# jisang93/VISinger

Hardware: AMD Instinct MI355X
Metric: audio samples/sec (22.05 kHz) + flow log-det rel-err, B=32 T_mel=1024 (higher is better)
Workload: dtype f32 (split-f16 x3 on the f16 MFMA, f32 accumulate); 1 GPU; VISinger synthesis (text-enc + pitch-pred + frame-prior + flow-inverse + HiFi-GAN), B=32/GPU T_mel=1024 hop=256 hidden=192 fp32 tensors, random-init weights; per_gpu_batch=32, global_batch=32, t_mel=1024, hop=256, hidden=192, parallelism=dp1 (utterance shard, no collective), streams=2

## Files before the change

visinger_amd/csrc/resblock_f16.hip:

```cpp
#include "conv_common.h"

#include <algorithm>
#include <type_traits>

namespace vs {

__device__ __forceinline__ unsigned max3_u32(unsigned a, unsigned b, unsigned c) {
    unsigned r;
    asm("v_max3_u32 %0, %1, %2, %3" : "=v"(r) : "v"(a), "v"(b), "v"(c));
    return r;
}

typedef float f32x4 __attribute__((ext_vector_type(4)));

#ifdef VS_RB_MFMA32
constexpr bool RB_MFMA16 = false;
#else
constexpr bool RB_MFMA16 = true;
#endif

constexpr int RB_MAXCONV = 6;
constexpr int RB_MAXPAD = 28;

struct ResblockParams {
    const float *x;
    long long x_bs;
    const void *ws[RB_MAXCONV];
    const float *bias[RB_MAXCONV];
    const float *wscale[RB_MAXCONV];
    int dil[RB_MAXCONV];
    float *y;
    const float *acc;
    long long y_bs, acc_bs;
    float scale;
    int B, C, T, K, nconv, nchunks;
    int H;
    int MP;
    int fast_epi;
    int bf16;
    unsigned long long *stamps;
};

__device__ __forceinline__ void rb_stamp(const ResblockParams &p, int slot) {
    if (p.stamps && threadIdx.x == 0) {
        const unsigned lin = blockIdx.x + gridDim.x * blockIdx.z;
        p.stamps[(size_t)lin * 64 + slot] = __builtin_amdgcn_s_memrealtime();
        p.stamps[(size_t)lin * 64 + 32 + slot] = __builtin_amdgcn_s_memtime();
    }
}

template <int NT_W, int WAVES_M, int WAVES_N, int MP, int PLANES, bool PB>
__device__ __forceinline__ void resblock_body(const ResblockParams &p) {
    constexpr int NW = WAVES_M * WAVES_N;
    static_assert(NW == 4 || NW == 8, "four or eight waves");
    static_assert(PLANES == 2 || (PLANES == 1), "two f16 planes or one bf16 plane");
    static_assert(!PB || PLANES == 1, "bf16-resident tensors go with the plain-bf16 arithmetic");
    constexpr int BN = 32 * NT_W * WAVES_N;
    constexpr int KG = 4 * WAVES_M;
    constexpr int WT = BN + 2 * MP;
    constexpr int TPL = KG * WT * 4;
    extern __shared__ __attribute__((aligned(16))) float smem[];
    unsigned *const Tb = reinterpret_cast<unsigned *>(smem);
    int *const smax = reinterpret_cast<int *>(Tb + PLANES * TPL);

    const int tid = threadIdx.x, lane = tid & 63;
    const int wave = __builtin_amdgcn_readfirstlane(tid >> 6);
    const int wm = wave % WAVES_M, wn = wave / WAVES_M;
    constexpr bool M16 = RB_MFMA16 && PLANES == 2;
    constexpr int NA = M16 ? 4 * NT_W : NT_W, AR = M16 ? 4 : 16;
    constexpr int NCT = M16 ? 2 * NT_W : NT_W, CTW = M16 ? 16 : 32;
    constexpr int RT = M16 ? 2 : 1;
    constexpr int KSTEP = M16 ? 32 : 16;
    using acc_t = std::conditional_t<M16, f32x4, f32x16>;
    auto ct_of = [](int a) { return M16 ? (a >> 1) : a; };
    const int lhalf = lane >> 5;
    const int lcol = lane & (CTW - 1);
    auto tile_col = [&](int a) { return ct_of(a) * CTW + lcol; };
    const int b = blockIdx.z;
    const int NOUT = BN - 2 * p.H;
    const int n0 = blockIdx.x * NOUT;
    const int t0 = n0 - p.H;
    const int KT = p.K;
    const int nch = p.nchunks / (KSTEP / 16);
    const int nsteps = nch * KT;
    auto tile_row = [&](int a, int r) { return M16 ? 16 * (a & 1) + 4 * (lane >> 4) + r : (r & 3) + 8 * (r >> 2) + 4 * lhalf; };

    rb_stamp(p, 0);
    for (int e = tid; e < PLANES * KG * 2 * MP; e += 64 * NW) {
        const int rowi = e / (2 * MP), c = e % (2 * MP);
        *reinterpret_cast<u32x4 *>(Tb + (rowi * WT + (c < MP ? c : BN + c)) * 4) = u32x4{0u, 0u, 0u, 0u};
    }

    bool inside[NCT];
    acc_t xr[NA], acc[NA];
    {
        const char *const xbase = reinterpret_cast<const char *>(p.x) + (long long)b * p.x_bs * (PB ? 2 : 4);
        const __amdgpu_buffer_rsrc_t xsrc =
            __builtin_amdgcn_make_buffer_rsrc((void *)xbase, 0, (int)((long long)p.C * p.T * (PB ? 2 : 4)), 0x00020000);
#pragma unroll
        for (int j = 0; j < NCT; ++j) {
            const int n = t0 + wn * (NT_W * 32) + j * CTW + lcol;
            inside[j] = (n >= 0) && (n < p.T);
        }
#pragma unroll
        for (int a = 0; a < NA; ++a) {
            const int nc = min(max(t0 + wn * (NT_W * 32) + tile_col(a), 0), p.T - 1);
#pragma unroll
            for (int r = 0; r < AR; ++r) {
                if constexpr (PB)
                    xr[a][r] = u2f((unsigned)(unsigned short)__builtin_amdgcn_raw_buffer_load_b16(xsrc, ((wm * 32 + tile_row(a, r)) * p.T + nc) * 2, 0, 0) << 16);
                else
                    xr[a][r] = __builtin_bit_cast(float, __builtin_amdgcn_raw_buffer_load_b32(xsrc, ((wm * 32 + tile_row(a, r)) * p.T + nc) * 4, 0, 0));
            }
        }
#pragma unroll
        for (int a = 0; a < NA; ++a)
#pragma unroll
            for (int r = 0; r < AR; ++r) xr[a][r] = inside[ct_of(a)] ? xr[a][r] : 0.f;
    }

    bool all_in = true;
#pragma unroll
    for (int j = 0; j < NCT; ++j) all_in = all_in && (__builtin_amdgcn_ballot_w64(inside[j]) == ~0ull);
    rb_stamp(p, 1);
    auto mma_step = [&](const u32x4 (&acur)[RT][PLANES], const unsigned *xs, auto zc_c) __attribute__((always_inline)) {
        constexpr bool ZC = decltype(zc_c)::value;
        const f32x16 zero16 = {0.f, 0.f, 0.f, 0.f, 0.f, 0.f, 0.f, 0.f, 0.f, 0.f, 0.f, 0.f, 0.f, 0.f, 0.f, 0.f};
        const f32x4 zero4 = {0.f, 0.f, 0.f, 0.f};
        u32x4 bf[PLANES], bn[PLANES];
#pragma unroll
        for (int pl = 0; pl < PLANES; ++pl) bf[pl] = *reinterpret_cast<const u32x4 *>(xs + pl * TPL);
#pragma unroll
        for (int j = 0; j < NCT; ++j) {
            if (j + 1 < NCT) {
#pragma unroll
                for (int pl = 0; pl < PLANES; ++pl) bn[pl] = *reinterpret_cast<const u32x4 *>(xs + pl * TPL + (j + 1) * (CTW * 4));
            }
            __builtin_amdgcn_sched_barrier(0);
            if constexpr (M16) {
                auto mm = [&](int ta, int tb) __attribute__((always_inline)) {
#pragma unroll
                    for (int rt = 0; rt < 2; ++rt)
                        acc[2 * j + rt] = __builtin_amdgcn_mfma_f32_16x16x32_f16(__builtin_bit_cast(f16x8, acur[rt][ta]), __builtin_bit_cast(f16x8, bf[tb]), acc[2 * j + rt], 0, 0, 0);
                };
                if constexpr (ZC) {
#pragma unroll
                    for (int rt = 0; rt < 2; ++rt)
                        acc[2 * j + rt] = __builtin_amdgcn_mfma_f32_16x16x32_f16(__builtin_bit_cast(f16x8, acur[rt][1]), __builtin_bit_cast(f16x8, bf[0]), zero4, 0, 0, 0);
                } else mm(1, 0);
                mm(0, 1); mm(0, 0);
            } else if constexpr (PLANES == 2) {
                auto mm = [&](int ta, int tb) __attribute__((always_inline)) {
                    acc[j] = __builtin_amdgcn_mfma_f32_32x32x16_f16(__builtin_bit_cast(f16x8, acur[0][ta]), __builtin_bit_cast(f16x8, bf[tb]), acc[j], 0, 0, 0);
                };
                if constexpr (ZC) acc[j] = __builtin_amdgcn_mfma_f32_32x32x16_f16(__builtin_bit_cast(f16x8, acur[0][1]), __builtin_bit_cast(f16x8, bf[0]), zero16, 0, 0, 0);
                else mm(1, 0);
                mm(0, 1); mm(0, 0);
            } else {
                acc[j] = __builtin_amdgcn_mfma_f32_32x32x16_bf16(__builtin_bit_cast(bf16x8, acur[0][0]), __builtin_bit_cast(bf16x8, bf[0]), ZC ? zero16 : acc[j], 0, 0, 0);
            }
            __builtin_amdgcn_sched_barrier(0);
#pragma unroll
            for (int pl = 0; pl < PLANES; ++pl) bf[pl] = bn[pl];
        }
    };

    for (int c = 0; c < p.nconv; ++c) {
        const bool second = (c & 1) != 0;
        int lane_c = lane;
        asm volatile("" : "+v"(lane_c));
        const int lh = lane_c >> 5, l5 = lane_c & (CTW - 1);
        unsigned mkey = 0u;
        typedef float f32x2 __attribute__((ext_vector_type(2)));
        const f32x2 slope2 = {0.1f, 0.1f};
        auto transform = [&](auto in_c) __attribute__((always_inline)) {
            constexpr bool ALL_IN = decltype(in_c)::value;
#pragma unroll
            for (int j = 0; j < NA; ++j)
#pragma unroll
                for (int r = 0; r < AR; r += 2) {
                    const f32x2 v2 = second ? f32x2{acc[j][r], acc[j][r + 1]} : f32x2{xr[j][r], xr[j][r + 1]};
                    const f32x2 t2 = v2 * slope2;
                    float v0 = fmaxf(v2.x, t2.x), v1 = fmaxf(v2.y, t2.y);
                    if constexpr (!ALL_IN) { v0 = inside[ct_of(j)] ? v0 : 0.f; v1 = inside[ct_of(j)] ? v1 : 0.f; }
                    acc[j][r] = v0;
                    acc[j][r + 1] = v1;
                    if constexpr (PLANES == 2) mkey = max3_u32(mkey, (f2u(v0) << 1) + 0x01000000u, (f2u(v1) << 1) + 0x01000000u);
                }
        };
        if (all_in) transform(std::true_type{});
        else transform(std::false_type{});
        int eb = 127;
        float sx = 1.f;
        if constexpr (PLANES == 2) {
            const int ebw = wave_max_u8(f16_key_exponent(mkey));
            int *const slot = smax + (c & 1) * NW;
            if (lane == 0) slot[wave] = ebw;
            __syncthreads();
            eb = max(max(max(slot[0], slot[1]), max(slot[2], slot[3])), F16_EB_MIN);
            if constexpr (NW == 8) eb = max(eb, max(max(slot[4], slot[5]), max(slot[6], slot[7])));
            sx = f16_scale(eb);
        } else {
            __syncthreads();
        }
        rb_stamp(p, 2 + 4 * c);
#pragma unroll
        for (int j = 0; j < NA; ++j) {
            const int col = MP + wn * (NT_W * 32) + ct_of(j) * CTW + l5;
#pragma unroll
            for (int g = 0; g < AR / 4; ++g) {
                unsigned d0[PLANES], d1[PLANES];
                if constexpr (PLANES == 2) {
                    const f32x2 sx2 = {sx, sx};
                    const f32x2 a0 = f32x2{acc[j][4 * g], acc[j][4 * g + 1]} * sx2, a1 = f32x2{acc[j][4 * g + 2], acc[j][4 * g + 3]} * sx2;
                    split_pair_h(a0.x, a0.y, d0);
                    split_pair_h(a1.x, a1.y, d1);
                } else {
                    split_pair<1>(acc[j][4 * g], acc[j][4 * g + 1], d0);
                    split_pair<1>(acc[j][4 * g + 2], acc[j][4 * g + 3], d1);
                }
                unsigned *dst = M16 ? Tb + ((wm * 4 + 2 * (j & 1) + lh) * WT + col) * 4 + ((lane_c >> 4) & 1) * 2 : Tb + ((wm * 4 + g) * WT + col) * 4 + lh * 2;
#pragma unroll
                for (int pl = 0; pl < PLANES; ++pl) *reinterpret_cast<uint2 *>(dst + pl * TPL) = make_uint2(d0[pl], d1[pl]);
            }
        }
        const int d = p.dil[c];
        const int pad = d * (KT - 1) / 2;
        const int lane_w = M16 ? (lane_c >> 5) * (PLANES * 64) + (lane_c & 15) + 32 * ((lane_c >> 4) & 1) : lane_c;
        const u32x4 *const wbase = reinterpret_cast<const u32x4 *>(p.ws[c]) + (long long)wm * KT * p.nchunks * (PLANES * 64) + lane_w;
        u32x4 a0[RT][PLANES], a1[RT][PLANES];
        const int a_dtap = p.nchunks * (PLANES * 64), a_dwrap = (KSTEP / 16) * (PLANES * 64) - (KT - 1) * a_dtap;
        const int a_last = ((KT - 1) * p.nchunks + (p.nchunks - KSTEP / 16)) * (PLANES * 64);
        int aoff = 0;
        auto load_a = [&](u32x4 (&dst)[RT][PLANES]) __attribute__((always_inline)) {
            const u32x4 *src = wbase + min(aoff, a_last);
#pragma unroll
            for (int rt = 0; rt < RT; ++rt)
#pragma unroll
                for (int pl = 0; pl < PLANES; ++pl) dst[rt][pl] = src[pl * 64 + rt * 16];
        };
        int pt = 0, tap = 0, s = 0;
        auto advance = [&]() __attribute__((always_inline)) { if (++pt == KT) { pt = 0; aoff += a_dwrap; } else aoff += a_dtap; };
        load_a(a0); advance();
        __syncthreads();
        rb_stamp(p, 3 + 4 * c);
        const unsigned *const xlane = Tb + ((M16 ? lane_c >> 4 : lh) * WT + MP + wn * (NT_W * 32) + l5 - pad) * 4;
        const int x_dtap = d * 4, x_dwrap = (KSTEP / 8) * WT * 4 - (KT - 1) * d * 4;
        int xoff = 0;
        auto step = [&](u32x4 (&acur)[RT][PLANES], u32x4 (&apre)[RT][PLANES], auto zc_c) __attribute__((always_inline)) {
            load_a(apre); advance();
            mma_step(acur, xlane + xoff, zc_c);
            if (++tap == KT) { tap = 0; xoff += x_dwrap; } else xoff += x_dtap;
            ++s;
        };
        step(a0, a1, std::true_type{});
        step(a1, a0, std::false_type{});
        while (s < nsteps) {
            step(a0, a1, std::false_type{});
            if (s < nsteps) step(a1, a0, std::false_type{});
        }
        rb_stamp(p, 4 + 4 * c);
        const float isx = (PLANES == 2) ? f16_inv_scale(eb) : 1.f, isw = (PLANES == 2) ? p.wscale[c][1] : 1.f;
        const float *const bias = p.bias[c] + wm * 32;
        const f32x2 isx2 = {isx, isx}, isw2 = {isw, isw};
        auto brow = [&](int rt, int r) { return M16 ? 16 * rt + 4 * (lane_c >> 4) + r : (r & 3) + 8 * (r >> 2) + 4 * lh; };
        if (second) {
#pragma unroll
            for (int rt = 0; rt < RT; ++rt)
#pragma unroll
                for (int r = 0; r < AR; r += 2) {
                    const f32x2 bv2 = {bias[brow(rt, r)], bias[brow(rt, r + 1)]};
#pragma unroll
                    for (int j = rt; j < NA; j += RT) {
                        const f32x2 a = {acc[j][r], acc[j][r + 1]};
                        const f32x2 v = __builtin_elementwise_fma(a * isx2, isw2, bv2);
                        f32x2 x2 = {xr[j][r], xr[j][r + 1]};
                        x2 += v;
                        xr[j][r] = x2.x; xr[j][r + 1] = x2.y;
                    }
                }
        } else {
#pragma unroll
            for (int rt = 0; rt < RT; ++rt)
#pragma unroll
                for (int r = 0; r < AR; r += 2) {
                    const f32x2 bv2 = {bias[brow(rt, r)], bias[brow(rt, r + 1)]};
#pragma unroll
                    for (int j = rt; j < NA; j += RT) {
                        const f32x2 a = {acc[j][r], acc[j][r + 1]};
                        const f32x2 v = __builtin_elementwise_fma(a * isx2, isw2, bv2);
                        acc[j][r] = v.x; acc[j][r + 1] = v.y;
                    }
                }
        }
        rb_stamp(p, 5 + 4 * c);
    }
    __syncthreads();

    int lane_e = lane;
    asm volatile("" : "+v"(lane_e));
    const int tile_row0 = wm * 32;
    const bool has_acc = p.acc != nullptr;
    float *const yb = p.y + (long long)b * p.y_bs;
    const float *const accp = has_acc ? p.acc + (long long)b * p.acc_bs : nullptr;
    unsigned short *const yh = reinterpret_cast<unsigned short *>(p.y) + (long long)b * p.y_bs;
    const unsigned short *const acch = reinterpret_cast<const unsigned short *>(p.acc) + (long long)b * p.acc_bs;
    if (p.fast_epi && (n0 + NOUT <= p.T)) {
        constexpr int CW = 32 * NT_W, LPR = CW / 4, RPI = 64 / LPR, RPP = M16 ? 16 : 8, NPS = 32 / RPP, NIT = RPP / RPI;
        float *const Lw = smem + wave * RPP * CW;
        const int lrow = lane_e / LPR, c4 = (lane_e % LPR) * 4;
        const int ctile = wn * CW + c4;
        const bool live = (ctile >= p.H) && (ctile < BN - p.H);
        const long long goff0 = (long long)(tile_row0 + lrow) * p.T + t0 + ctile;
        float4 a4[NPS][NIT];
        if (live && has_acc) {
#pragma unroll
            for (int ps = 0; ps < NPS; ++ps)
#pragma unroll
                for (int it = 0; it < NIT; ++it) {
                    if constexpr (PB) a4[ps][it] = bf4_to_f4(*reinterpret_cast<const uint2 *>(acch + goff0 + (long long)(RPP * ps + it * RPI) * p.T));
                    else a4[ps][it] = *reinterpret_cast<const float4 *>(accp + goff0 + (long long)(RPP * ps + it * RPI) * p.T);
                }
        }
#pragma unroll
        for (int ps = 0; ps < NPS; ++ps) {
#pragma unroll
            for (int q = 0; q < 4; ++q)
#pragma unroll
                for (int j = 0; j < NCT; ++j) {
                    if constexpr (M16) Lw[(q + 4 * (lane_e >> 4)) * CW + 16 * j + (lane_e & 15)] = xr[2 * j + ps][q];
                    else Lw[(q + 4 * (lane_e >> 5)) * CW + 32 * j + (lane_e & 31)] = xr[j][4 * ps + q];
                }
            if (live) {
#pragma unroll
                for (int it = 0; it < NIT; ++it) {
                    float4 v = *reinterpret_cast<const float4 *>(Lw + (it * RPI + lrow) * CW + c4);
                    if (has_acc) { v.x += a4[ps][it].x; v.y += a4[ps][it].y; v.z += a4[ps][it].z; v.w += a4[ps][it].w; }
                    if (p.scale != 1.f) { v.x *= p.scale; v.y *= p.scale; v.z *= p.scale; v.w *= p.scale; }
                    if constexpr (PB) *reinterpret_cast<uint2 *>(yh + goff0 + (long long)(RPP * ps + it * RPI) * p.T) = f4_to_bf4(v);
                    else *reinterpret_cast<float4 *>(yb + goff0 + (long long)(RPP * ps + it * RPI) * p.T) = v;
                }
            }
        }
    } else {
#pragma unroll
        for (int j = 0; j < NA; ++j) {
            const int ctile = wn * (NT_W * 32) + tile_col(j);
            const int n = t0 + ctile;
            const bool okc = (ctile >= p.H) && (ctile < BN - p.H) && (n < p.T);
            const int nc = min(max(n, 0), p.T - 1);
#pragma unroll
            for (int r = 0; r < AR; ++r) {
                const long long off = (long long)(tile_row0 + tile_row(j, r)) * p.T + nc;
                float v = xr[j][r];
                if constexpr (PB) {
                    if (has_acc) v += u2f((unsigned)acch[off] << 16);
                    v *= p.scale;
                    if (okc) yh[off] = (unsigned short)(rne_bf16(v) >> 16);
                } else {
                    if (has_acc) v += accp[off];
                    v *= p.scale;
                    if (okc) yb[off] = v;
                }
            }
        }
    }
    if (p.stamps) {
        __builtin_amdgcn_s_waitcnt(0);
        rb_stamp(p, 2 + 4 * p.nconv);
    }
}

template <int NT_W, int WAVES_M, int WAVES_N, int MP>
__global__ void __launch_bounds__(64 * WAVES_M * WAVES_N, NT_W == 2 ? 4 : 2) resblock_f16_kernel(const ResblockParams p) {
    resblock_body<NT_W, WAVES_M, WAVES_N, MP, 2, false>(p);
}

template <int NT_W, int WAVES_M, int WAVES_N, int MP>
__global__ void __launch_bounds__(64 * WAVES_M * WAVES_N, 2) resblock_bf16_kernel(const ResblockParams p) {
    resblock_body<NT_W, WAVES_M, WAVES_N, MP, 1, true>(p);
}

static int margin_of(int maxpad) { return maxpad <= 8 ? 8 : (maxpad <= 16 ? 16 : RB_MAXPAD); }

template <int NT_W, int WAVES_M, int WAVES_N>
static size_t resblock_lds(int MP, int planes = 2) {
    constexpr int BN = 32 * NT_W * WAVES_N, KG = 4 * WAVES_M;
    return std::max<size_t>((size_t)planes * KG * (BN + 2 * MP) * 16 + 64, (size_t)WAVES_M * WAVES_N * (RB_MFMA16 && planes == 2 ? 16 : 8) * (32 * NT_W) * sizeof(float));
}

template <int NT_W, int WAVES_M, int WAVES_N, int MP, bool BF>
static int launch_resblock_mp(const ResblockParams &p, hipStream_t s) {
    constexpr int BN = 32 * NT_W * WAVES_N;
    auto kern = BF ? resblock_bf16_kernel<NT_W, WAVES_M, WAVES_N, MP> : resblock_f16_kernel<NT_W, WAVES_M, WAVES_N, MP>;
    const size_t lds = resblock_lds<NT_W, WAVES_M, WAVES_N>(MP, BF ? 1 : 2);
    static bool attr_set = false;
    if (!attr_set) {
        VS_CHECK_HIP(hipFuncSetAttribute((const void *)kern, hipFuncAttributeMaxDynamicSharedMemorySize, 160 * 1024));
        attr_set = true;
    }
    dim3 grid((unsigned)ceil_div(p.T, BN - 2 * p.H), 1, (unsigned)p.B);
    hipLaunchKernelGGL(kern, grid, dim3(64 * WAVES_M * WAVES_N), lds, s, p);
    VS_CHECK_HIP(hipGetLastError());
    set_last_kernel(BF ? "resblock_bf16_kernel<%d, %d, %d, %d>" : "resblock_f16_kernel<%d, %d, %d, %d>", NT_W, WAVES_M, WAVES_N, MP);
    return VS_OK;
}

template <int NT_W, int WAVES_M, int WAVES_N, bool BF>
static int launch_resblock_margin(const ResblockParams &p, hipStream_t s) {
    switch (margin_of(p.MP)) {
        case 8: return launch_resblock_mp<NT_W, WAVES_M, WAVES_N, 8, BF>(p, s);
        case 16: return launch_resblock_mp<NT_W, WAVES_M, WAVES_N, 16, BF>(p, s);
        default: return launch_resblock_mp<NT_W, WAVES_M, WAVES_N, RB_MAXPAD, BF>(p, s);
    }
}

template <int NT_W, int WAVES_M, int WAVES_N>
static int launch_resblock_cfg(const ResblockParams &p, hipStream_t s) {
    return p.bf16 ? launch_resblock_margin<NT_W, WAVES_M, WAVES_N, true>(p, s) : launch_resblock_margin<NT_W, WAVES_M, WAVES_N, false>(p, s);
}

}

using namespace vs;

extern unsigned long long *g_stamp_buf;

extern "C" {

int vs_resblock_supported(vs_conv_t *const *convs, int nconv) {
    if (!convs || nconv < 2 || nconv > RB_MAXCONV || (nconv & 1)) return 0;
    const vs_conv *c0 = convs[0];
    if (!c0) return 0;
    const int C = c0->c_in, k = c0->k;
    if (!(C == 32 || C == 64 || C == 128) || !(k & 1) || k < 3 || k > 11) return 0;
    if (c0->math != VS_MATH_SPLIT3 && c0->math != VS_MATH_BF16) return 0;
    const int planes = c0->math == VS_MATH_BF16 ? 1 : 2;
    int H = 0, MP = 0;
    for (int i = 0; i < nconv; ++i) {
        const vs_conv *c = convs[i];
        if (!c || c->kind != VS_CONV1D || c->c_in != C || c->c_out != C || c->k != k || c->flags != 0 || c->math != c0->math) return 0;
        if (c->pad != c->dil * (k - 1) / 2 || c->pad > RB_MAXPAD) return 0;
        H += c->pad;
        MP = std::max(MP, c->pad);
    }
    H = (H + 3) & ~3;
    if (C == 128)
        return 256 - 2 * H >= 64 && resblock_lds<4, 4, 2>(margin_of(MP), planes) <= 160 * 1024;
    return 256 - 2 * H >= 64;
}

int vs_resblock_forward(vs_conv_t *const *convs, int nconv, const vs_conv_io_t *io, void *stream) {
    VS_REQUIRE(convs && io, "vs_resblock_forward: NULL argument");
    VS_REQUIRE(vs_resblock_supported(convs, nconv), "vs_resblock_forward: unsupported chain of convs (32 / 64 / 128 channels, one odd k <= 11, VS_MATH_SPLIT3, "
                                                   "'same' padding, an even number of convs <= 6)");
    VS_REQUIRE(io->x && io->out[0].y && io->B > 0 && io->B <= 65535 && io->T > 0, "vs_resblock_forward: bad io");
    const bool bf = convs[0]->math == VS_MATH_BF16;
    VS_REQUIRE(io->x_dtype == (bf ? VS_DTYPE_BF16 : VS_DTYPE_F32) && io->y_dtype == io->x_dtype,
               "vs_resblock_forward: fp32 tensors with VS_MATH_SPLIT3, bf16-resident tensors with VS_MATH_BF16");
    VS_REQUIRE(io->in_act == VS_IN_LRELU && !io->mask && !io->bias_b && !io->split_row && io->out[0].mode == VS_OUT_LINEAR &&
                   io->out[0].out_act == VS_OUT_NONE && !io->out[0].out_mask && !io->out[0].res,
               "vs_resblock_forward: only the unmasked leaky-relu residual form is fused (the residual input is x itself)");
    ResblockParams p;
    memset(&p, 0, sizeof(p));
    const vs_conv *c0 = convs[0];
    const int C = c0->c_in;
    p.bf16 = bf;
    VS_REQUIRE((long long)C * io->T * 4 < (1ll << 31), "vs_resblock_forward: item exceeds the 2 GiB buffer-descriptor range");
    const long long dflt = (long long)C * io->T;
    p.x = static_cast<const float *>(io->x); p.x_bs = io->x_bs ? io->x_bs : dflt;
    int H = 0;
    for (int i = 0; i < nconv; ++i) {
        const vs_conv *c = convs[i];
        VS_REQUIRE(c->weights_set, "vs_resblock_forward: weights not set");
        p.ws[i] = c->ws.p; p.bias[i] = c->biasp.as<float>(); p.wscale[i] = c->wsc.as<float>(); p.dil[i] = c->dil;
        H += c->pad;
        p.MP = std::max(p.MP, c->pad);
    }
    p.H = (H + 3) & ~3;
    const vs_conv_out_t &o = io->out[0];
    p.y = static_cast<float *>(o.y); p.acc = static_cast<const float *>(o.acc);
    p.y_bs = o.y_bs ? o.y_bs : dflt; p.acc_bs = o.acc_bs ? o.acc_bs : dflt;
    p.scale = (o.scale == 0.f) ? 1.f : o.scale;
    p.B = (int)io->B; p.C = C; p.T = (int)io->T; p.K = c0->k; p.nconv = nconv; p.nchunks = c0->nchunks;
    p.stamps = g_stamp_buf;
    auto al16 = [](const void *q) { return (reinterpret_cast<uintptr_t>(q) & 15u) == 0; };
    auto al8 = [](const void *q) { return (reinterpret_cast<uintptr_t>(q) & 7u) == 0; };
    p.fast_epi = (io->T % 4 == 0) && (p.y_bs % 4 == 0) && (!p.acc || p.acc_bs % 4 == 0) &&
                 (bf ? al8(p.y) && (!p.acc || al8(p.acc)) : al16(p.y) && (!p.acc || al16(p.acc)));
    hipStream_t s = as_stream(stream);
    if (C == 32) {
        if (opt(OPT_RB_TILE256) || p.H <= 12 || 512 - 2 * p.H > io->T + 256) return launch_resblock_cfg<2, 1, 4>(p, s);
        return launch_resblock_cfg<4, 1, 4>(p, s);
    }
    if (C == 128) {
        if (nconv == 2 && 128 - 2 * p.H >= 64 && 2 * (resblock_lds<4, 4, 1>(margin_of(p.MP), bf ? 1 : 2) + 64) <= 160 * 1024)
            return launch_resblock_cfg<4, 4, 1>(p, s);
        return launch_resblock_cfg<4, 4, 2>(p, s);
    }
#ifndef VS_RB_NO_WIDE64
    if (p.H >= 20 && (long long)ceil_div(p.T, 512 - 2 * p.H) * p.B >= 512 && !opt(OPT_RB_TILE256) &&
        resblock_lds<4, 2, 4>(margin_of(p.MP), bf ? 1 : 2) <= 160 * 1024)
        return launch_resblock_cfg<4, 2, 4>(p, s);
#endif
    return launch_resblock_cfg<4, 2, 2>(p, s);
}

}
```

Baseline: 132.6 million audio samples/s.

## Add halo-trimmed resblock tiles and f32 abs-max exponent key

Adds an optional TRIM mode (off unless VS_RB_TRIM is defined) that tracks which column tiles stay valid as receptive-field halos shrink across the dilated convs. It skips MFMAs, transforms and LDS stores for tiles that have gone out of range, and zeroes tiles that just became invalid. The per-wave exponent reduction for f16 split scaling now uses v_max3_f32 on absolute values by default when NT_W==2. It falls back to a finite-only rescan when the max is inf or NaN. This replaces the integer key trick, at the cost of a rare slow path.

```diff
diff --git a/visinger_amd/csrc/resblock_f16.hip b/visinger_amd/csrc/resblock_f16.hip
--- a/visinger_amd/csrc/resblock_f16.hip
+++ b/visinger_amd/csrc/resblock_f16.hip
@@ -11,12 +11,28 @@
     return r;
 }
 
+__device__ __forceinline__ float max3_abs_f32(float m, float a, float b) {
+    float r;
+    asm("v_max3_f32 %0, %1, |%2|, |%3|" : "=v"(r) : "v"(m), "v"(a), "v"(b));
+    return r;
+}
+
 typedef float f32x4 __attribute__((ext_vector_type(4)));
 
 #ifdef VS_RB_MFMA32
 constexpr bool RB_MFMA16 = false;
 #else
 constexpr bool RB_MFMA16 = true;
+#endif
+#ifdef VS_RB_TRIM
+constexpr bool RB_TRIM = true;
+#else
+constexpr bool RB_TRIM = false;
+#endif
+#ifdef VS_RB_KEY_U32
+constexpr bool RB_KEY_F32 = false;
+#else
+constexpr bool RB_KEY_F32 = true;
 #endif
 
 constexpr int RB_MAXCONV = 6;
@@ -123,10 +139,45 @@
 #pragma unroll
     for (int j = 0; j < NCT; ++j) all_in = all_in && (__builtin_amdgcn_ballot_w64(inside[j]) == ~0ull);
     rb_stamp(p, 1);
+    constexpr bool TRIM = RB_TRIM && M16 && MP > 8 && NT_W == 4;
+    constexpr unsigned ALL_TILES = (1u << NCT) - 1u;
+    unsigned in_mask = ALL_TILES, out_mask = ALL_TILES;
+    int p_sum = 0;
     auto mma_step = [&](const u32x4 (&acur)[RT][PLANES], const unsigned *xs, auto zc_c) __attribute__((always_inline)) {
         constexpr bool ZC = decltype(zc_c)::value;
         const f32x16 zero16 = {0.f, 0.f, 0.f, 0.f, 0.f, 0.f, 0.f, 0.f, 0.f, 0.f, 0.f, 0.f, 0.f, 0.f, 0.f, 0.f};
         const f32x4 zero4 = {0.f, 0.f, 0.f, 0.f};
+        if constexpr (TRIM) {
+            u32x4 bq[2][PLANES];
+            if (out_mask & 1u) {
+#pragma unroll
+                for (int pl = 0; pl < PLANES; ++pl) bq[0][pl] = *reinterpret_cast<const u32x4 *>(xs + pl * TPL);
+            }
+#pragma unroll
+            for (int j = 0; j < NCT; ++j) {
+                if (j + 1 < NCT && (out_mask & (2u << j))) {
+#pragma unroll
+                    for (int pl = 0; pl < PLANES; ++pl) bq[(j + 1) & 1][pl] = *reinterpret_cast<const u32x4 *>(xs + pl * TPL + (j + 1) * (CTW * 4));
+                }
+                __builtin_amdgcn_sched_barrier(0);
+                if (out_mask & (1u << j)) {
+                    const u32x4 (&bt)[PLANES] = bq[j & 1];
+                    auto mm = [&](int ta, int tb) __attribute__((always_inline)) {
+#pragma unroll
+                        for (int rt = 0; rt < 2; ++rt)
+                            acc[2 * j + rt] = __builtin_amdgcn_mfma_f32_16x16x32_f16(__builtin_bit_cast(f16x8, acur[rt][ta]), __builtin_bit_cast(f16x8, bt[tb]), acc[2 * j + rt], 0, 0, 0);
+                    };
+                    if constexpr (ZC) {
+#pragma unroll
+                        for (int rt = 0; rt < 2; ++rt)
+                            acc[2 * j + rt] = __builtin_amdgcn_mfma_f32_16x16x32_f16(__builtin_bit_cast(f16x8, acur[rt][1]), __builtin_bit_cast(f16x8, bt[0]), zero4, 0, 0, 0);
+                    } else mm(1, 0);
+                    mm(0, 1); mm(0, 0);
+                }
+                __builtin_amdgcn_sched_barrier(0);
+            }
+            return;
+        }
         u32x4 bf[PLANES], bn[PLANES];
 #pragma unroll
         for (int pl = 0; pl < PLANES; ++pl) bf[pl] = *reinterpret_cast<const u32x4 *>(xs + pl * TPL);
@@ -167,16 +218,27 @@
 
     for (int c = 0; c < p.nconv; ++c) {
         const bool second = (c & 1) != 0;
+        unsigned zero_mask = 0u;
+        if constexpr (TRIM) {
+            if (c > 0) { zero_mask = in_mask & ~out_mask; in_mask = out_mask; }
+            p_sum += p.dil[c] * (KT - 1) / 2;
+            const int skip = p_sum >> 4;
+            const int lo = min(max(skip - wn * NCT, 0), NCT), hi = min(max(BN / 16 - skip - wn * NCT, 0), NCT);
+            out_mask = ((1u << hi) - 1u) & ~((1u << lo) - 1u);
+        }
         int lane_c = lane;
         asm volatile("" : "+v"(lane_c));
         const int lh = lane_c >> 5, l5 = lane_c & (CTW - 1);
         unsigned mkey = 0u;
+        float mabs = 0.f;
         typedef float f32x2 __attribute__((ext_vector_type(2)));
         const f32x2 slope2 = {0.1f, 0.1f};
+        constexpr bool KEY_F32 = RB_KEY_F32 && NT_W == 2;
         auto transform = [&](auto in_c) __attribute__((always_inline)) {
             constexpr bool ALL_IN = decltype(in_c)::value;
 #pragma unroll
-            for (int j = 0; j < NA; ++j)
+            for (int j = 0; j < NA; ++j) {
+                if constexpr (TRIM) { if (!(in_mask & (1u << ct_of(j)))) continue; }
 #pragma unroll
                 for (int r = 0; r < AR; r += 2) {
                     const f32x2 v2 = second ? f32x2{acc[j][r], acc[j][r + 1]} : f32x2{xr[j][r], xr[j][r + 1]};
@@ -185,15 +247,32 @@
                     if constexpr (!ALL_IN) { v0 = inside[ct_of(j)] ? v0 : 0.f; v1 = inside[ct_of(j)] ? v1 : 0.f; }
                     acc[j][r] = v0;
                     acc[j][r + 1] = v1;
-                    if constexpr (PLANES == 2) mkey = max3_u32(mkey, (f2u(v0) << 1) + 0x01000000u, (f2u(v1) << 1) + 0x01000000u);
-                }
+                    if constexpr (PLANES == 2 && KEY_F32) mabs = max3_abs_f32(mabs, v0, v1);
+                    else if constexpr (PLANES == 2) mkey = max3_u32(mkey, (f2u(v0) << 1) + 0x01000000u, (f2u(v1) << 1) + 0x01000000u);
+                }
+            }
         };
         if (all_in) transform(std::true_type{});
         else transform(std::false_type{});
         int eb = 127;
         float sx = 1.f;
         if constexpr (PLANES == 2) {
-            const int ebw = wave_max_u8(f16_key_exponent(mkey));
+            int ebw;
+            if constexpr (KEY_F32) {
+                ebw = wave_max_u8((int)(f2u(mabs) >> 23));
+                if (ebw == 255) {
+                    float mfin = 0.f;
+#pragma unroll
+                    for (int j = 0; j < NA; ++j) {
+                        if constexpr (TRIM) { if (!(in_mask & (1u << ct_of(j)))) continue; }
+#pragma unroll
+                        for (int r = 0; r < AR; ++r) { const float av = __builtin_fabsf(acc[j][r]); mfin = __builtin_fmaxf(mfin, av < __builtin_inff() ? av : 0.f); }
+                    }
+                    ebw = wave_max_u8((int)(f2u(mfin) >> 23));
+                }
+            } else {
+                ebw = wave_max_u8(f16_key_exponent(mkey));
+            }
             int *const slot = smax + (c & 1) * NW;
             if (lane == 0) slot[wave] = ebw;
             __syncthreads();
@@ -207,6 +286,16 @@
 #pragma unroll
         for (int j = 0; j < NA; ++j) {
             const int col = MP + wn * (NT_W * 32) + ct_of(j) * CTW + l5;
+            if constexpr (TRIM) {
+                if (!(in_mask & (1u << ct_of(j)))) {
+                    if (zero_mask & (1u << ct_of(j))) {
+                        unsigned *dst = Tb + ((wm * 4 + 2 * (j & 1) + lh) * WT + col) * 4 + ((lane_c >> 4) & 1) * 2;
+#pragma unroll
+                        for (int pl = 0; pl < PLANES; ++pl) *reinterpret_cast<uint2 *>(dst + pl * TPL) = make_uint2(0u, 0u);
+                    }
+                    continue;
+                }
+            }
 #pragma unroll
             for (int g = 0; g < AR / 4; ++g) {
                 unsigned d0[PLANES], d1[PLANES];
@@ -264,7 +353,33 @@
         const float *const bias = p.bias[c] + wm * 32;
         const f32x2 isx2 = {isx, isx}, isw2 = {isw, isw};
         auto brow = [&](int rt, int r) { return M16 ? 16 * rt + 4 * (lane_c >> 4) + r : (r & 3) + 8 * (r >> 2) + 4 * lh; };
-        if (second) {
+        if constexpr (TRIM) {
+            f32x2 bvt[RT][AR / 2];
+#pragma unroll
+            for (int rt = 0; rt < RT; ++rt)
+#pragma unroll
+                for (int r = 0; r < AR; r += 2) bvt[rt][r / 2] = f32x2{bias[brow(rt, r)], bias[brow(rt, r + 1)]};
+            auto scale_out = [&](auto second_c) __attribute__((always_inline)) {
+#pragma unroll
+                for (int j = 0; j < NA; ++j) {
+                    if (!(out_mask & (1u << ct_of(j)))) continue;
+#pragma unroll
+                    for (int r = 0; r < AR; r += 2) {
+                        const f32x2 a = {acc[j][r], acc[j][r + 1]};
+                        const f32x2 v = __builtin_elementwise_fma(a * isx2, isw2, bvt[j % RT][r / 2]);
+                        if constexpr (decltype(second_c)::value) {
+                            f32x2 x2 = {xr[j][r], xr[j][r + 1]};
+                            x2 += v;
+                            xr[j][r] = x2.x; xr[j][r + 1] = x2.y;
+                        } else {
+                            acc[j][r] = v.x; acc[j][r + 1] = v.y;
+                        }
+                    }
+                }
+            };
+            if (second) scale_out(std::true_type{});
+            else scale_out(std::false_type{});
+        } else if (second) {
 #pragma unroll
             for (int rt = 0; rt < RT; ++rt)
 #pragma unroll
```

New measurement: 132.6 million audio samples/s. About the same (-0.0%).
